# lzhangbj/ASVA

Measured on AMD Instinct MI355X. Metric: UNet denoising steps/sec, 12x256x256 bf16, CFG on, higher is better.
Workload: dtype bf16; 1 GPU; BASELINE configs[1]: AVSync15 shape, 1 clip(s) per GPU per forward, 12x256x256 (latent 12x32x32), SD1.5-shaped AudioUNet3D 1.17B params random-init, CFG batch 2 (audio guidance 4.0), DDIM-50 schedule, step = UNet forward + guidance + scheduler update; clips_per_gpu=1, unet_batch=2, frames=12, launch=hipGraph replay, parallelism=dp1 (independent clips)

## Files before the change

asva_amd/_lib.py:

```python
from __future__ import annotations

import ctypes as C
import os

import torch

from . import precision as P

_HERE = os.path.dirname(os.path.abspath(__file__))
LIB_PATH = os.environ.get("AVSD_LIB_PATH") or os.path.join(_HERE, "libavsd_hip.so")
LIB_PATHS = {"bf16": LIB_PATH, "fp16": os.environ.get("AVSD_LIB_PATH_F16") or os.path.join(_HERE, "libavsd_hip_f16.so")}

c_void_p, c_int, c_float, c_int64 = C.c_void_p, C.c_int, C.c_float, C.c_int64


class GemmDesc(C.Structure):

    _fields_ = [
        ("A", c_void_p), ("A2", c_void_p), ("W", c_void_p), ("out", c_void_p),
        ("bias", c_void_p), ("rowvec", c_void_p), ("res1", c_void_p), ("res2", c_void_p),
        ("M", C.c_int32), ("N", C.c_int32), ("K", C.c_int32),
        ("lda", C.c_int32), ("lda2", C.c_int32), ("k_split", C.c_int32), ("ldw", C.c_int32),
        ("ldc", C.c_int32), ("ldr1", C.c_int32), ("ldr2", C.c_int32),
        ("rows_per_vec", C.c_int32), ("ldv", C.c_int32),
# ... 40 lines not shown
    "avsd_gemm_bf16": (c_int, [C.POINTER(GemmDesc), c_void_p]),
    "avsd_sizeof_gemm_desc": (c_int, []),
    "avsd_cross_attention_block": (c_int, [C.POINTER(XAttnDesc), c_void_p]),
    "avsd_gemm_conv3r_supported": (c_int, [c_int, c_int, c_int, c_int]),
    "avsd_gemm_conv3r2d_supported": (c_int, [c_int, c_int, c_int, c_int]),
    "avsd_cross_attention_block_supported": (c_int, [c_int, c_int, c_int]),
    "avsd_sizeof_xattn_desc": (c_int, []),
    "avsd_qproj_attention": (c_int, [C.POINTER(XAttnDesc), c_void_p]),
    "avsd_qproj_attention_supported": (c_int, [c_int, c_int, c_int, c_int]),
    "avsd_ff_block": (c_int, [c_void_p, c_int, c_void_p, c_int, c_float, c_void_p, c_void_p, c_void_p, c_void_p, c_void_p, c_void_p, c_void_p,
                              c_void_p, c_int, c_void_p, c_int, c_int, c_int, c_void_p]),
    "avsd_ff_block_supported": (c_int, [c_int, c_int, c_int]),
    "avsd_temporal_block": (c_int, [c_void_p, c_int, c_void_p, c_int, c_float, c_void_p, c_void_p, c_void_p, c_void_p, c_void_p, c_void_p,
                                    c_void_p, c_int, c_void_p, c_int, c_int, c_int, c_int, c_int, c_float, c_void_p]),
    "avsd_temporal_block_supported": (c_int, [c_int, c_int, c_int, c_int]),
    "avsd_linear_small_m": (c_int, [c_void_p, c_void_p, c_void_p, c_void_p, c_int, c_int, c_int, c_int, c_int, c_int, c_void_p]),
    "avsd_groupnorm_stats": (c_int, [c_void_p, c_int, c_int, c_void_p, c_int, c_int, c_int, c_int, c_int, c_void_p, c_int, c_void_p]),
    "avsd_groupnorm_apply": (c_int, [c_void_p, c_int, c_int, c_void_p, c_int, c_int, c_int, c_int, c_int, c_void_p, c_void_p, c_float,
                                     c_void_p, c_int, c_int, c_void_p, c_int, c_void_p]),
    "avsd_ln_fold": (c_int, [c_void_p, c_int, c_int, c_void_p, c_void_p]),
    "avsd_groupnorm_fused_supported": (c_int, [c_int, c_int, c_int, c_int, c_int, c_int]),
    "avsd_groupnorm_fused": (c_int, [c_void_p, c_int, c_int, c_void_p, c_int, c_int, c_int, c_int, c_int, c_void_p, c_void_p, c_float,
                                     c_int, c_void_p, c_int, c_void_p]),
    "avsd_groupnorm_nchunks": (c_int, [c_int, c_int, c_int]),
    "avsd_groupnorm_scratch_floats": (c_int, [c_int, c_int, c_int, c_int]),
    "avsd_layernorm": (c_int, [c_void_p, c_int, c_void_p, c_int, c_int, c_int, c_void_p, c_void_p, c_float, c_void_p, c_int, c_int, c_void_p]),
    "avsd_softmax_rows": (c_int, [c_void_p, c_int, c_void_p, c_int, c_int, c_int, c_void_p]),
    "avsd_attention": (c_int, [c_void_p, c_int, c_void_p, c_int, c_void_p, c_int, c_void_p, c_int, c_int, c_int, c_int, c_int,
                               c_int, c_int, c_int, c_void_p, c_int, c_float, c_void_p]),
    "avsd_attention_fp8": (c_int, [c_void_p, c_int, c_void_p, c_int, c_void_p, c_int, c_void_p, c_int, c_int, c_int, c_int, c_int,
# ... 129 lines not shown
```

asva_amd/build.py:

```python
from __future__ import annotations

import os
import subprocess
import sys
from concurrent.futures import ThreadPoolExecutor

HERE = os.path.dirname(os.path.abspath(__file__))
CSRC = os.path.join(HERE, "csrc")
OBJ = os.path.join(CSRC, "_obj")
LIB = os.path.join(HERE, "libavsd_hip.so")
VARIANTS = {"bf16": ("", LIB, []), "fp16": ("_f16", os.path.join(HERE, "libavsd_hip_f16.so"), ["-DAVSD_F16=1"])}
SOURCES = ["lib.hip", "attention.hip", "attention_x2.hip", "gemm_f32.hip", "gemm4.hip", "nstream.hip", "conv3r.hip", "norm.hip", "groupnorm_fused.hip", "elementwise.hip", "audio.hip", "xattn.hip", "qattn.hip", "ffblock.hip", "tblock.hip", "attention_fp8.hip", "avsync.hip", "clip_text.hip", "imagebind_eval.hip", "jpeg.hip", "loss.hip", "plan.hip"]
GEMM_UNITS = 7
HEADERS = [os.path.join(CSRC, "avsd_common.h"), os.path.join(CSRC, "gemm_common.h"), os.path.join(CSRC, "gemm4_loops.inc"), os.path.join(CSRC, "band_units.h"),
           os.path.join(HERE, "..", "include", "avsd.h")]
FLAGS = ["--offload-arch=gfx950", "-O3", "-std=c++17", "-fPIC", "-Wall", "-Wno-unused-function"]


PLAN_HOST = os.path.join(HERE, "plan_host")


def _hipcc() -> str:
    for cand in (os.environ.get("HIPCC"), "/opt/rocm/bin/hipcc", "hipcc"):
        if cand and (os.path.isabs(cand) and os.path.exists(cand) or not os.path.isabs(cand)):
            return cand
    raise RuntimeError("hipcc not found")

# ... 57 lines not shown
```

asva_amd/csrc/plan.hip:

```cpp
#include "avsd_common.h"

#include <stdio.h>
#include <string.h>

#include <string>
#include <type_traits>
#include <utility>
#include <vector>

namespace {

struct RArg {
  int64_t i = 0;
  double f = 0.0;
  void* p = nullptr;
};

template <class T>
T conv(const RArg& a) {
  if constexpr (std::is_pointer_v<T>) return reinterpret_cast<T>(a.p);
  else if constexpr (std::is_floating_point_v<T>) return static_cast<T>(a.f);
  else return static_cast<T>(a.i);
}
template <class... A, size_t... I>
// ... 14 lines not shown
  const char* name;
  thunk_t thunk;
  size_t desc_bytes;
};
#define AVSD_PLAN_ENTRY(fn) {#fn, [](const RArg* a, int n) { return call(&fn, a, n, #fn); }, 0}
#define AVSD_PLAN_ENTRY_DESC(fn, T) {#fn, [](const RArg* a, int n) { return call(&fn, a, n, #fn); }, sizeof(T)}
const Entry kEntries[] = {
    AVSD_PLAN_ENTRY_DESC(avsd_gemm_bf16, avsd_gemm_desc), AVSD_PLAN_ENTRY_DESC(avsd_cross_attention_block, avsd_xattn_desc), AVSD_PLAN_ENTRY(avsd_linear_small_m),
    AVSD_PLAN_ENTRY(avsd_groupnorm_stats),  AVSD_PLAN_ENTRY(avsd_groupnorm_apply),       AVSD_PLAN_ENTRY(avsd_layernorm),
    AVSD_PLAN_ENTRY(avsd_softmax_rows),     AVSD_PLAN_ENTRY(avsd_attention),             AVSD_PLAN_ENTRY(avsd_attention_fp8),
    AVSD_PLAN_ENTRY(avsd_temporal_attention), AVSD_PLAN_ENTRY(avsd_ncfhw_to_rows),       AVSD_PLAN_ENTRY(avsd_rows_to_ncfhw),
    AVSD_PLAN_ENTRY(avsd_timestep_embedding), AVSD_PLAN_ENTRY(avsd_guided_step),         AVSD_PLAN_ENTRY(avsd_vae_postprocess),
    AVSD_PLAN_ENTRY(avsd_vae_postprocess_u8), AVSD_PLAN_ENTRY(avsd_kaldi_fbank),         AVSD_PLAN_ENTRY(avsd_patchify),
    AVSD_PLAN_ENTRY(avsd_vit_tokens),       AVSD_PLAN_ENTRY(avsd_copy),                  AVSD_PLAN_ENTRY(avsd_xattn_pack_kv),
    AVSD_PLAN_ENTRY_DESC(avsd_qproj_attention, avsd_xattn_desc), AVSD_PLAN_ENTRY(avsd_ff_block), AVSD_PLAN_ENTRY(avsd_temporal_block),
    AVSD_PLAN_ENTRY(avsd_linear_small_m_x2), AVSD_PLAN_ENTRY(avsd_groupnorm_stats_x2),   AVSD_PLAN_ENTRY(avsd_groupnorm_apply_x2),
    AVSD_PLAN_ENTRY(avsd_layernorm_x2),     AVSD_PLAN_ENTRY(avsd_attention_x2),          AVSD_PLAN_ENTRY(avsd_temporal_attention_x2),
    AVSD_PLAN_ENTRY(avsd_ncfhw_to_rows_x2), AVSD_PLAN_ENTRY(avsd_split_f32),             AVSD_PLAN_ENTRY(avsd_vae_postprocess_x2),
    AVSD_PLAN_ENTRY(avsd_vae_postprocess_u8_x2), AVSD_PLAN_ENTRY(avsd_softmax_rows_x2),
    AVSD_PLAN_ENTRY(avsd_groupnorm_fused),  AVSD_PLAN_ENTRY(avsd_groupnorm_fused_x2),
    AVSD_PLAN_ENTRY(avsd_ln_fold),          AVSD_PLAN_ENTRY(avsd_guided_multistep),      AVSD_PLAN_ENTRY(avsd_guided_unipc),
    AVSD_PLAN_ENTRY(avsd_window_turnover),
    AVSD_PLAN_ENTRY(avsd_convnd_f32),       AVSD_PLAN_ENTRY(avsd_maxpool_hw_f32),        AVSD_PLAN_ENTRY(avsd_mean_rows_f32),
    AVSD_PLAN_ENTRY(avsd_resize_aa_normalize_f32),
    AVSD_PLAN_ENTRY(avsd_convnd_ld_f32),    AVSD_PLAN_ENTRY(avsd_pool3_hw_f32),
    AVSD_PLAN_ENTRY(avsd_conv3d_same_f32),  AVSD_PLAN_ENTRY(avsd_maxpool3d_same_f32),
    AVSD_PLAN_ENTRY(avsd_embed_tokens_f32), AVSD_PLAN_ENTRY(avsd_layernorm_f32),         AVSD_PLAN_ENTRY(avsd_attention_causal_f32),
    AVSD_PLAN_ENTRY(avsd_quick_gelu_f32),
    AVSD_PLAN_ENTRY(avsd_attention_f32),    AVSD_PLAN_ENTRY(avsd_gelu_f32),              AVSD_PLAN_ENTRY(avsd_vit_tokens_f32),
    AVSD_PLAN_ENTRY(avsd_cosine_rows_f32),   AVSD_PLAN_ENTRY(avsd_normalize_rows_f32),
// ... 376 lines not shown
```

asva_amd/ops.py:

```python
from __future__ import annotations

import os
import ctypes as C
from typing import Optional, Tuple

import torch

from . import _lib
from . import precision as P
from ._lib import GemmDesc, XAttnDesc, check

PLAIN, TMIX, CONV3 = 0, 1, 2
GEGLU, OUT_F32, GELU, XCD_N, ROWSTATS, LNFUSE, RES1_F32, RES2_F32, X2, KROT, W_FRAG, OUT_REST = 1, 2, 4, 8, 16, 32, 64, 128, 256, 512, 1024, 2048
_XCD_MODE = "auto"
F32 = torch.float32


class KernelTimer:

    def __init__(self):
        self.records = []
        self.replays = []

    def start(self):
# ... 760 lines not shown
    M, K = x.shape
    N = w.shape[0]
    if not x.is_contiguous():
        raise ValueError("linear_small_m: x must be contiguous")
    if out is None:
        out = torch.empty((M, N), dtype=F32, device=x.device)
    if P.SPLIT:
        check(_lib.lib().avsd_linear_small_m_x2(_p(x), _p(w), _lo(w), _p(bias), _p(out), M, N, K, _ld(w), int(act_in), int(act_out),
                                                _stream()), "avsd_linear_small_m_x2")
        return out
    check(_lib.lib().avsd_linear_small_m(_p(x), _p(w), _p(bias), _p(out), M, N, K, _ld(w), int(act_in), int(act_out),
                                         _stream()), "avsd_linear_small_m")
    return out


_GN_FUSED = True

def groupnorm(x1: torch.Tensor, x2: Optional[torch.Tensor], nb: int, rows_per_batch: int, groups: int,
              gamma: torch.Tensor, beta: torch.Tensor, eps: float, act: bool,
              out: Optional[torch.Tensor] = None) -> torch.Tensor:
    _req(x1, P.ACT, "x1")
    c1 = x1.shape[1]
    c2 = 0
    if x2 is not None:
        _req(x2, P.ACT, "x2")
        c2 = x2.shape[1]
    _req(gamma, F32, "gamma")
    _req(beta, F32, "beta")
    L = _lib.lib()
    rows = nb * rows_per_batch
    if out is None:
# ... 321 lines not shown
    if out is None:
        out = torch.empty((M, Cc), dtype=P.ACT, device=h.device)
    _req(out, P.ACT, "out")
    if out.shape != (M, Cc):
        raise ValueError("temporal_block: out must be [M, C]")
    if scale is None:
        scale = float(Cc // heads) ** -0.5
    a_ = (_p(h), _ld(h), _p(stats), int(stats.shape[1]), float(eps), _p(wqkv_frag), _p(qkv_colsum), _p(qkv_bias), _p(posw), _p(wo_frag),
          _p(bo), _p(out), _ld(out), _p(rowstats), b, frames, hw, Cc, heads, float(scale))
    _timed("temporal_block", 8.0 * M * Cc * Cc + 4.0 * M * frames * Cc, _nbytes(h, out, rowstats) + 2.0 * (nq + Cc) * Cc,
           (h, stats, wqkv_frag, qkv_colsum, qkv_bias, posw, wo_frag, bo, rowstats, out),
           lambda: check(_lib.lib().avsd_temporal_block(*a_, _stream()), "avsd_temporal_block"))
    return out


def temporal_attention(qkv: torch.Tensor, *, b: int, frames: int, hw: int, heads: int,
                       scale: Optional[float] = None, out: Optional[torch.Tensor] = None) -> torch.Tensor:
    _req(qkv, P.ACT, "qkv")
    Cc = qkv.shape[1] // 3
    d = Cc // heads
    if out is None:
        out = alloc16((qkv.shape[0], Cc), qkv.device)
    if scale is None:
        scale = float(d) ** -0.5
    if P.SPLIT:
        a_ = (_p(qkv), _ld(qkv), _lo(qkv), _p(out), _ld(out), _lo(out), b, frames, hw, heads, d, float(scale))
        call = lambda: check(_lib.lib().avsd_temporal_attention_x2(*a_, _stream()), "avsd_temporal_attention_x2")
    else:
        a_ = (_p(qkv), _ld(qkv), _p(out), _ld(out), b, frames, hw, heads, d, float(scale))
        call = lambda: check(_lib.lib().avsd_temporal_attention(*a_, _stream()), "avsd_temporal_attention")
# ... 711 lines not shown
```

asva_amd/plan.py:

```python
from __future__ import annotations

import contextlib
import ctypes as C
import os
import struct
from typing import Dict, List, Optional, Tuple

import torch

from . import _lib
from . import precision as P

CONST, INPUT, OUTPUT = 1, 2, 3
MAGIC = b"AVSDPLN1"
_NOT_RECORDED = {"avsd_abi_version", "avsd_precision", "avsd_last_error", "avsd_device_info", "avsd_sizeof_gemm_desc",
                 "avsd_sizeof_xattn_desc", "avsd_cross_attention_block_supported", "avsd_qproj_attention_supported", "avsd_ff_block_supported", "avsd_temporal_block_supported", "avsd_groupnorm_nchunks",
                 "avsd_groupnorm_scratch_floats", "avsd_groupnorm_fused_supported", "avsd_gemm_conv3r_supported", "avsd_gemm_conv3r2d_supported"}


def _ptr_fields(struct_type) -> List[Tuple[str, int]]:
    return [(name, getattr(struct_type, name).offset) for name, tp in struct_type._fields_ if tp is C.c_void_p]


class _Proxy:

    def __init__(self, real, sink):
        self._real, self._sink = real, sink

    def __getattr__(self, name):
        fn = getattr(self._real, name)
        if (name in _NOT_RECORDED or name.startswith("avsd_plan_") or name.startswith("avsd_unet_") or name == "avsd_vae_decode"
# ... 237 lines not shown
```

asva_amd/unet.py:

```python
from __future__ import annotations

import inspect
import json
import math
import os
from typing import Any, Dict, Optional, Tuple, Union

import torch
from torch import nn

from . import precision as P

from . import ops
from .conditioning import mask_to_key_index
from .weights import Blob, _Pk, _Ref, from_act, group_qkv, pack_conv1x1, pack_device, pack_frag, pack_geglu, pack_linear, subpixel_ups, to_act, to_planes

CONFIG_NAME = "config.json"
SAFETENSORS_NAME = "diffusion_pytorch_model.safetensors"
BIN_NAME = "diffusion_pytorch_model.bin"

DOWN_TYPES = ("FFSpatioAudioTempCrossAttnDownBlock3D", "FFSpatioTempCrossAttnDownBlock3D", "FFSpatioTempResDownBlock3D")
UP_TYPES = ("FFSpatioAudioTempCrossAttnUpBlock3D", "FFSpatioTempCrossAttnUpBlock3D", "FFSpatioTempResUpBlock3D")
MID_TYPES = ("FFSpatioAudioTempCrossAttnUNetMidBlock3D", "FFSpatioTempCrossAttnUNetMidBlock3D")


_FUSE_LN = True
_FUSE_LN_TEMP = True
_F32_RES = os.environ.get("AVSD_F32_RESIDUAL", "0") != "0"
_ATTN_FP8 = os.environ.get("AVSD_ATTN_FP8", "0") != "0"
_FUSE_XATTN = True
_FUSE_QATTN = os.environ.get("AVSD_FUSE_QATTN", "1") != "0"
_FUSE_FF = os.environ.get("AVSD_FUSE_FF", "1") != "0"
_FUSE_TATTN = os.environ.get("AVSD_FUSE_TATTN", "1") != "0"
_LN_PREFOLD = True
_SHARE_PREFIX = True
_F32_CONV_Y = True


def _replicate(a: "_Act", r: int) -> "_Act":
    return _Act(ops.copy(a.lo, rep=r), None if a.hi is None else ops.copy(a.hi, rep=r),
                None if a.rest is None else ops.copy(a.rest, rep=r))


def _xa_fill(kv: torch.Tensor, n_kv: int, rows: int, C: int, idx: Optional[torch.Tensor], old=None):
    nb, lk = (n_kv, rows) if idx is None else (n_kv * idx.shape[0], idx.shape[1])
    lkp = (lk + 31) // 32 * 32
    if lkp > 96 or P.SPLIT:
        return None
# ... 308 lines not shown
                w1_ln=reg(w1_ln), b1_ln=reg(b1_ln), s1_ln=reg(from_act(w1_ln).sum(1)),
                norm_temp=self.aff(b.norm_temp), attn_temp=self.attn(b.attn_temp, True, b.norm_temp),
                pos1=self.lin(b.pos_embedding_temp.linear_1), pos2=self.lin(b.pos_embedding_temp.linear_2),
                norm3=self.aff(b.norm3), w1=reg(w1), b1=reg(b1), ff2=self.lin(b.ff.net[2]),
                dim=m.proj_in.weight.shape[0], audio=hasattr(b, "attn_audio"))
        if w1_ln.shape[1] in (320, 640) and not P.SPLIT:
            p.w1_ln_f = reg(pack_frag(w1_ln))
            if p.dim == 320:
                p.w2_f = reg(pack_frag(self.items[p.ff2.w.idx]))
                p.wp_f = reg(pack_frag(self.items[p.proj_out.w.idx]))
        if p.dim == 320 and not P.SPLIT:
            at = p.attn_temp
            at.wqkv_f = reg(pack_frag(group_qkv(self.items[at.wqkv_ln.idx])))
            at.sqkv_f, at.bqkv_f = reg(group_qkv(self.items[at.sqkv_ln.idx])), reg(group_qkv(self.items[at.bqkv_ln.idx]))
            at.wo_f = reg(pack_frag(self.items[at.wo.idx]))
        if p.audio:
            p.norm_audio = self.aff(b.norm_audio)
            p.attn_audio = self.attn(b.attn_audio, False, b.norm_audio)
        return p

    def block(self, m: _Block, where: Optional[str] = None):
        return _Pk(resnets=[self.res(r, where) for r in m.resnets],
                   attentions=[self.tr(a) for a in m.attentions] if hasattr(m, "attentions") else None,
                   down=self.ffconv(m.downsamplers[0].conv, "sampler", where) if hasattr(m, "downsamplers") else None,
                   up=self.ffconv(m.upsamplers[0].conv, "sampler", where, subpixel=P.SUBPIXEL_UPS) if hasattr(m, "upsamplers") else None)

    def finish(self, pk: _Pk, device, meta: bool = False) -> _Pk:
        if self.temb_w:
            pk.temb_w = self.reg(pack_linear(torch.cat(self.temb_w, 0)))
            pk.temb_b = self.reg(torch.cat(self.temb_b, 0))
# ... 556 lines not shown
        assert skip is None
        s = x
    tv = st.temb[:, p.temb_off:p.temb_off + p.cout]
    a = ops.groupnorm(x.lo, None if skip is None else skip.lo, st.B, rows_b, st.groups, p.norm1.g, p.norm1.b, st.eps, True)
    h = _ffconv(st, _Act(a), p.conv1, hw, temb=tv, master=False)
    a2 = ops.groupnorm(h.lo, None, st.B, rows_b, st.groups, p.norm2.g, p.norm2.b, st.eps, True)
    return _ffconv(st, _Act(a2), p.conv2, hw, res=s, rest=rest)


def _transformer(st, x: _Act, p, hw, heads, split: int = 1, rest=False) -> _Act:
    B, Fr = st.B, st.F
    L = hw[0] * hw[1]
    C = p.dim
    c = st.cond.blocks[st.tr_i]
    st.tr_i += 1
    n = ops.groupnorm(x.lo, None, B * Fr, L, st.groups, p.norm.g, p.norm.b, 1e-6, False)
    fused = C % 32 == 0 and st.fuse_ln
    eps = 1e-5
    M = B * Fr * L
    stats = [torch.empty((M, C // 32, 2), dtype=torch.float32, device=n.device) for _ in range(2)] if fused else None
    si = 0

    def stream(a, w, bias, res, want_stats=True, stats_pos=None, rest=False):
        nonlocal si
        m = _master(st, a, w.shape[0])
        if fused and want_stats:
            si ^= 1
            return _Act(ops.gemm(a, w, bias=bias, res1=None if res is None else res.res, rowstats=stats[si], master=m, stats_pos=stats_pos), m)
        o16 = o16r = None
        if rest and m is not None:
            o16, o16r = ops.alloc_planes((a.shape[0], w.shape[0]), a.device)
        return _Act(ops.gemm(a, w, bias=bias, res1=None if res is None else res.res, master=m, out=o16, out_rest=o16r), m, o16r)

    def cross(h, a, norm, xa, want_stats, unfused, stats_pos=None):
        nonlocal si
        if fused and st.fp8 is None and xa is not None and ops.cross_attention_block_supported(C, heads, xa.k.shape[1], M, L):
# ... 7 lines not shown
                                            heads=heads, L=L, q_per_kv=xa.q_per_kv, eps=eps, rowstats=s_out, master=m, stats_pos=stats_pos)
            return _Act(out, m)
        qa_ok = getattr(ops, "qproj_attention_supported", None)
        if (_FUSE_QATTN and fused and st.fp8 is None and xa is not None and qa_ok is not None
                and qa_ok(C, heads, xa.k.shape[1], M, L, xa.q_per_kv)):
            o = ops.qproj_attention(h.lo, stats[si], a.wq_ln, a.sq_ln, a.bq_ln, xa.k, xa.vt, xa.lk, heads=heads, L=L,
                                    q_per_kv=xa.q_per_kv, eps=eps)
            return stream(o, a.wo, a.bo, h, want_stats=want_stats, stats_pos=stats_pos)
        return stream(unfused(), a.wo, a.bo, h, want_stats=want_stats, stats_pos=stats_pos)

    def proj(h, norm, wl, bl, sl, w_plain):
        if fused:
            return ops.gemm(h.lo, wl, bias=bl, ln=(stats[si], sl, eps))
        return ops.gemm(ops.layernorm(h.lo, norm.g, norm.b), w_plain)

    h = stream(n, p.proj_in.w, p.proj_in.b, None)
    a1 = p.attn1
    if fused:
        kv = ops.gemm_batched(h.lo.view(B, Fr * L, C)[:, :L], a1.wkv_ln.unsqueeze(0).expand(B, 2 * C, C), bias=a1.bkv_ln,
                              ln=(stats[si], a1.skv_ln, eps)).view(B * L, 2 * C)
        q = ops.gemm(h.lo, a1.wq_ln, bias=a1.bq_ln, ln=(stats[si], a1.sq_ln, eps))
    else:
        n1 = ops.layernorm(h.lo, p.norm1.g, p.norm1.b)
        q = ops.gemm(n1, a1.wq)
        kv = ops.gemm_batched(n1.view(B, Fr * L, C)[:, :L], a1.wkv.unsqueeze(0).expand(B, 2 * C, C)).view(B * L, 2 * C)
    o = ops.attention(q, kv[:, :C], kv[:, C:], bq=B * Fr, lq=L, lk=L, kv_rows=L, heads=heads, q_per_kv=Fr, frames=Fr, fp8=st.fp8)
    h = stream(o, a1.wo, a1.bo, h)
    if split > 1:
        h, x = _replicate(h, split), _replicate(x, split)
        st.B = B = B * split
        M = B * Fr * L
        if fused:
            cur = stats[si]
            stats = [torch.empty((M, C // 32, 2), dtype=torch.float32, device=n.device) for _ in range(2)]
            ops.copy(cur, stats[si], rep=split)
    if p.audio:
        aa = p.attn_audio

        def audio_attention():
            q = proj(h, p.norm_audio, getattr(aa, "wq_ln", None), getattr(aa, "bq_ln", None), getattr(aa, "sq_ln", None), aa.wq)
            idx = st.cond.key_index
            return ops.attention(q, c.audio_kv[:, :C], c.audio_kv[:, C:], bq=B * Fr, lq=L,
                                 lk=idx.shape[1] if idx is not None else c.audio_len, kv_rows=c.audio_len, heads=heads,
                                 q_per_kv=Fr if c.audio_pf == 1 else 1, frames=st.cond.idx_frames if idx is not None else Fr,
                                 key_index=idx, fp8=st.fp8)

        h = cross(h, aa, p.norm_audio, getattr(c, "xa_audio", None), True, audio_attention)
    a2 = p.attn2

# ... 42 lines not shown
```

include/avsd.h:

```cpp
#ifndef AVSD_H
#define AVSD_H

#include <stddef.h>
#include <stdint.h>

#ifdef __cplusplus
extern "C" {
#endif

#define AVSD_OK 0
#define AVSD_EINVAL (-1)
#define AVSD_ELAUNCH (-2)
#define AVSD_ENODEV (-3)

#define AVSD_ABI_VERSION 10

int avsd_abi_version(void);
const char* avsd_precision(void);
const char* avsd_last_error(void);
int avsd_device_info(char* name_host, int len, int* num_cu_host);

enum { AVSD_GEMM_PLAIN = 0, AVSD_GEMM_TMIX = 1, AVSD_GEMM_CONV3 = 2 };
enum { AVSD_GEMM_GEGLU = 1, AVSD_GEMM_OUT_F32 = 2, AVSD_GEMM_GELU = 4, AVSD_GEMM_XCD_N = 8, AVSD_GEMM_ROWSTATS = 16,
       AVSD_GEMM_LNFUSE = 32, AVSD_GEMM_RES1_F32 = 64, AVSD_GEMM_RES2_F32 = 128, AVSD_GEMM_X2 = 256, AVSD_GEMM_KROT = 512, AVSD_GEMM_W_FRAG = 1024,
// ... 74 lines not shown
int avsd_sizeof_xattn_desc(void);

int avsd_qproj_attention_supported(int C, int heads, int lk_pad, int rows_per_kv_block);
int avsd_qproj_attention(const avsd_xattn_desc* desc_host, void* stream);

int avsd_ff_block_supported(int M, int C, int with_proj_out);
int avsd_ff_block(const void* h, int ldh, const float* ln_stats, int ln_nblk, float ln_eps, const void* w1_frag, const float* w1_colsum,
                  const float* b1, const void* w2_frag, const float* b2, const void* wp_frag, const float* bp, const void* x, int ldx,
                  void* out, int ldo, int M, int C, void* stream);

int avsd_temporal_block_supported(int M, int C, int heads, int frames);
int avsd_temporal_block(const void* h, int ldh, const float* ln_stats, int ln_nblk, float ln_eps, const void* wqkv_frag,
                        const float* qkv_colsum, const float* qkv_bias, const float* posw, const void* wo_frag, const float* bo,
                        void* out, int ldo, float* rowstats, int B, int frames, int hw, int C, int heads, float scale, void* stream);

int avsd_linear_small_m(const float* x, const void* W_bf16, const float* bias, float* out,
                        int M, int N, int K, int ldw, int act_in, int act_out, void* stream);

int avsd_groupnorm_stats(const void* x1, int ld1, int c1, const void* x2, int ld2, int c2,
                         int nb, int rows_per_batch, int groups, float* scratch, int nchunks, void* stream);
int avsd_groupnorm_apply(const void* x1, int ld1, int c1, const void* x2, int ld2, int c2,
                         int nb, int rows_per_batch, int groups, const float* gamma, const float* beta, float eps,
                         const float* scratch, int nchunks, int act, void* y, int ldy, void* stream);
int avsd_groupnorm_fused_supported(int nb, int rows_per_batch, int groups, int c1, int c2, int split);
int avsd_groupnorm_fused(const void* x1, int ld1, int c1, const void* x2, int ld2, int c2, int nb, int rows_per_batch,
                         int groups, const float* gamma, const float* beta, float eps, int act, void* y, int ldy, void* stream);
int avsd_groupnorm_nchunks(int nb, int rows_per_batch, int channels);
int avsd_groupnorm_scratch_floats(int nb, int nchunks, int groups, int channels);

int avsd_ln_fold(const float* stats, int M, int nblk, float* out, void* stream);
// ... 182 lines not shown
```

Baseline: 92.89 steps/s.

## Fuse groupnorm apply, proj_in and LN-folded Q projection into one kernel

```diff
diff --git a/asva_amd/_lib.py b/asva_amd/_lib.py
--- a/asva_amd/_lib.py
+++ b/asva_amd/_lib.py
@@ -78,6 +78,9 @@
     "avsd_temporal_block": (c_int, [c_void_p, c_int, c_void_p, c_int, c_float, c_void_p, c_void_p, c_void_p, c_void_p, c_void_p, c_void_p,
                                     c_void_p, c_int, c_void_p, c_int, c_int, c_int, c_int, c_int, c_float, c_void_p]),
     "avsd_temporal_block_supported": (c_int, [c_int, c_int, c_int, c_int]),
+    "avsd_block_front": (c_int, [c_void_p, c_int, c_void_p, c_int, c_void_p, c_void_p, c_float, c_int, c_int, c_void_p, c_void_p, c_void_p,
+                                 c_void_p, c_void_p, c_float, c_void_p, c_int, c_void_p, c_void_p, c_int, c_int, c_int, c_void_p]),
+    "avsd_block_front_supported": (c_int, [c_int, c_int, c_int, c_int, c_int]),
     "avsd_linear_small_m": (c_int, [c_void_p, c_void_p, c_void_p, c_void_p, c_int, c_int, c_int, c_int, c_int, c_int, c_void_p]),
     "avsd_groupnorm_stats": (c_int, [c_void_p, c_int, c_int, c_void_p, c_int, c_int, c_int, c_int, c_int, c_void_p, c_int, c_void_p]),
     "avsd_groupnorm_apply": (c_int, [c_void_p, c_int, c_int, c_void_p, c_int, c_int, c_int, c_int, c_int, c_void_p, c_void_p, c_float,
diff --git a/asva_amd/build.py b/asva_amd/build.py
--- a/asva_amd/build.py
+++ b/asva_amd/build.py
@@ -10,7 +10,7 @@
 OBJ = os.path.join(CSRC, "_obj")
 LIB = os.path.join(HERE, "libavsd_hip.so")
 VARIANTS = {"bf16": ("", LIB, []), "fp16": ("_f16", os.path.join(HERE, "libavsd_hip_f16.so"), ["-DAVSD_F16=1"])}
-SOURCES = ["lib.hip", "attention.hip", "attention_x2.hip", "gemm_f32.hip", "gemm4.hip", "nstream.hip", "conv3r.hip", "norm.hip", "groupnorm_fused.hip", "elementwise.hip", "audio.hip", "xattn.hip", "qattn.hip", "ffblock.hip", "tblock.hip", "attention_fp8.hip", "avsync.hip", "clip_text.hip", "imagebind_eval.hip", "jpeg.hip", "loss.hip", "plan.hip"]
+SOURCES = ["lib.hip", "attention.hip", "attention_x2.hip", "gemm_f32.hip", "gemm4.hip", "nstream.hip", "conv3r.hip", "norm.hip", "groupnorm_fused.hip", "elementwise.hip", "audio.hip", "xattn.hip", "qattn.hip", "ffblock.hip", "tblock.hip", "fblock.hip", "attention_fp8.hip", "avsync.hip", "clip_text.hip", "imagebind_eval.hip", "jpeg.hip", "loss.hip", "plan.hip"]
 GEMM_UNITS = 7
 HEADERS = [os.path.join(CSRC, "avsd_common.h"), os.path.join(CSRC, "gemm_common.h"), os.path.join(CSRC, "gemm4_loops.inc"), os.path.join(CSRC, "band_units.h"),
            os.path.join(HERE, "..", "include", "avsd.h")]
diff --git a/asva_amd/csrc/fblock.hip b/asva_amd/csrc/fblock.hip
--- /dev/null
+++ b/asva_amd/csrc/fblock.hip
@@ -0,0 +1,320 @@
+#include "gemm_common.h"
+
+namespace {
+
+typedef unsigned u32x4b __attribute__((ext_vector_type(4)));
+
+struct fb_args {
+  const h16_t* x; int ldx;
+  const float* partial; int nchunks;
+  const float* gamma; const float* beta; float gn_eps;
+  int rpb;
+  const u32x4b* wpi; const float* bpi;
+  const u32x4b* wq; const float* q_colsum; const float* q_bias; float ln_eps;
+  h16_t* h; int ldh;
+  float* rowstats;
+  h16_t* q; int ldq;
+  int M;
+};
+
+constexpr int FR_C = 320, FR_G = 32, FR_CG = FR_C / FR_G, FR_RF = 3, FR_BM = 32 * FR_RF;
+constexpr int FR_KS = FR_C / 16;
+constexpr int FR_NBLK = FR_C / 32;
+constexpr int FR_MIN_RPB = 8, FR_MAXB = (FR_BM - 2) / FR_MIN_RPB + 2;
+constexpr int FR_PITCH = FR_C * 2 + 16;
+constexpr int FR_BAND = FR_BM * FR_PITCH;
+constexpr int FR_TABLE = FR_MAXB * 2 * FR_C * 4;
+constexpr int FR_STATS = FR_BM * FR_NBLK * 8;
+constexpr int FR_MR = FR_MAXB * FR_G * 8;
+constexpr size_t FR_LDS = (size_t)2 * FR_BAND + FR_STATS + FR_MR;
+static_assert(FR_MAXB == 13 && FR_TABLE <= FR_BAND && FR_BAND % 16 == 0 && FR_LDS <= 160 * 1024, "LDS carve");
+
+__device__ __forceinline__ void unit_pack(const float (&v)[16], uint4& lo, uint4& hi) {
+  unsigned x[2][2], y[2][2];
+#pragma unroll
+  for (int d = 0; d < 2; ++d) {
+    const auto e = __builtin_amdgcn_permlane32_swap(pack2h(v[0 + 2 * d], v[1 + 2 * d]), pack2h(v[8 + 2 * d], v[9 + 2 * d]), false, false);
+    const auto o = __builtin_amdgcn_permlane32_swap(pack2h(v[4 + 2 * d], v[5 + 2 * d]), pack2h(v[12 + 2 * d], v[13 + 2 * d]), false, false);
+    x[0][d] = e[0]; x[1][d] = e[1];
+    y[0][d] = o[0]; y[1][d] = o[1];
+  }
+  lo = make_uint4(x[0][0], x[0][1], x[1][0], x[1][1]);
+  hi = make_uint4(y[0][0], y[0][1], y[1][0], y[1][1]);
+}
+
+__global__ __launch_bounds__(512, 1) void fblock_kernel(const fb_args p) {
+  extern __shared__ __attribute__((aligned(16))) unsigned char smb[];
+  constexpr int KS = FR_KS, PITCH = FR_PITCH, RF = FR_RF;
+  constexpr int D2 = 4;
+  const int tid = threadIdx.x, lane = tid & 63;
+  const int wave = __builtin_amdgcn_readfirstlane(tid >> 6);
+  const int m0 = blockIdx.x * FR_BM;
+  unsigned char* const band_n = smb;
+  unsigned char* const band_h = smb + FR_BAND;
+  float* const table = reinterpret_cast<float*>(band_h);
+  float2* const lstats = reinterpret_cast<float2*>(smb + 2 * FR_BAND);
+  float2* const mr = reinterpret_cast<float2*>(smb + 2 * FR_BAND + FR_STATS);
+  const int c0 = wave;
+  const bool extra = wave < 6;
+  const int c1 = extra ? 8 + wave / 3 : 8, b1 = extra ? wave % 3 : 0;
+  const int bat0 = m0 / p.rpb;
+  const int nbat = min(m0 + FR_BM - 1, p.M - 1) / p.rpb - bat0 + 1;
+
+  u32x4b qa[D2], qb[D2];
+  auto prefetch = [&](const u32x4b* w, int ln) {
+    const u32x4b* wa = w + ln + (int64_t)c0 * KS * 64;
+    const u32x4b* wb = w + ln + (int64_t)c1 * KS * 64;
+#pragma unroll
+    for (int d = 0; d < D2; ++d) {
+      qa[d] = __builtin_nontemporal_load(wa + d * 64);
+      if (extra) qb[d] = __builtin_nontemporal_load(wb + d * 64);
+    }
+  };
+  prefetch(p.wpi, lane);
+  constexpr int V = FR_C / 8;
+  constexpr int NV = (FR_BM * V + 511) / 512;
+  uint4 xv[NV];
+#pragma unroll
+  for (int i = 0; i < NV; ++i) {
+    const int v = min(tid + i * 512, FR_BM * V - 1), r = v / V, c = v - r * V;
+    xv[i] = *reinterpret_cast<const uint4*>(p.x + (int64_t)min(m0 + r, p.M - 1) * p.ldx + c * 8);
+  }
+  {
+    const int sub = tid & 31, half = tid >> 5;
+    const int npair = nbat * FR_G;
+    const float2* part = reinterpret_cast<const float2*>(p.partial);
+    for (int p0 = 0; p0 < npair; p0 += 64) {
+      float2 u[4][2];
+      const float2* base[4];
+#pragma unroll
+      for (int j = 0; j < 4; ++j) {
+        const int pi = min(p0 + 16 * j + half, npair - 1), t = pi / FR_G, g = pi - t * FR_G;
+        base[j] = part + (int64_t)(bat0 + t) * p.nchunks * FR_G + g;
+#pragma unroll
+        for (int e = 0; e < 2; ++e) {
+          const int k = sub + 32 * e;
+          u[j][e] = k < p.nchunks ? base[j][(int64_t)k * FR_G] : make_float2(0.f, 0.f);
+        }
+      }
+#pragma unroll
+      for (int j = 0; j < 4; ++j) {
+        const int pi = p0 + 16 * j + half;
+        double a = 0.0, q = 0.0;
+#pragma unroll
+        for (int e = 0; e < 2; ++e)
+          if (sub + 32 * e < p.nchunks) { a += (double)u[j][e].x; q += (double)u[j][e].y; }
+        for (int k = sub + 64; k < p.nchunks; k += 32) {
+          const float2 w = base[j][(int64_t)k * FR_G];
+          a += (double)w.x;
+          q += (double)w.y;
+        }
+        for (int off = 16; off > 0; off >>= 1) {
+          a += __shfl_xor(a, off, 64);
+          q += __shfl_xor(q, off, 64);
+        }
+        if (sub == 0 && pi < npair) {
+          const double n = (double)p.rpb * FR_CG;
+          const double mean = a / n;
+          double var = q / n - mean * mean;
+          if (var < 0.0) var = 0.0;
+          mr[pi] = make_float2((float)mean, (float)(1.0 / sqrt(var + (double)p.gn_eps)));
+        }
+      }
+    }
+  }
+  __syncthreads();
+  for (int i = tid; i < nbat * FR_C; i += 512) {
+    const int t = i / FR_C, c = i - t * FR_C;
+    const float2 s = mr[t * FR_G + c / FR_CG];
+    const float smean = s.x, srstd = s.y;
+    const float sc = srstd * p.gamma[c];
+    table[t * 2 * FR_C + c] = sc;
+    table[t * 2 * FR_C + FR_C + c] = p.beta[c] - smean * sc;
+  }
+  __syncthreads();
+#pragma unroll
+  for (int i = 0; i < NV; ++i) {
+    const int v = tid + i * 512, r = v / V, c = v - r * V;
+    if (v < FR_BM * V) {
+      const float* ss = table + (min(m0 + r, p.M - 1) / p.rpb - bat0) * 2 * FR_C + c * 8;
+      const float4 s0 = *reinterpret_cast<const float4*>(ss), s1 = *reinterpret_cast<const float4*>(ss + 4);
+      const float4 h0 = *reinterpret_cast<const float4*>(ss + FR_C), h1 = *reinterpret_cast<const float4*>(ss + FR_C + 4);
+      const float sc[8] = {s0.x, s0.y, s0.z, s0.w, s1.x, s1.y, s1.z, s1.w};
+      const float sh[8] = {h0.x, h0.y, h0.z, h0.w, h1.x, h1.y, h1.z, h1.w};
+      float f[8];
+      unpack8(xv[i], f);
+#pragma unroll
+      for (int e = 0; e < 8; ++e) f[e] = fmaf(f[e], sc[e], sh[e]);
+      *reinterpret_cast<uint4*>(band_n + r * PITCH + c * 16) = pack8(f);
+    }
+  }
+  __syncthreads();
+
+  f32x16 acc[4];
+  auto project = [&](const unsigned char* band, const u32x4b* w, int ln) {
+    const unsigned char* arow = band + (ln & 31) * PITCH + (ln >> 5) * 16;
+    const unsigned char* arow1 = arow + b1 * 32 * PITCH;
+    const u32x4b* wa = w + ln + (int64_t)c0 * KS * 64;
+    const u32x4b* wb = w + ln + (int64_t)c1 * KS * 64;
+#pragma unroll
+    for (int u = 0; u < 4; ++u)
+#pragma unroll
+      for (int r = 0; r < 16; ++r) acc[u][r] = 0.f;
+#pragma unroll
+    for (int ks = 0; ks < KS; ++ks) {
+      __builtin_amdgcn_sched_barrier(0);
+      h16x8 hf[RF];
+#pragma unroll
+      for (int b = 0; b < RF; ++b) hf[b] = *reinterpret_cast<const h16x8*>(arow + b * 32 * PITCH + ks * 32);
+      const h16x8 wf = __builtin_bit_cast(h16x8, qa[ks % D2]);
+#pragma unroll
+      for (int b = 0; b < RF; ++b) acc[b] = mfma32x32x16(wf, hf[b], acc[b], 0, 0, 0);
+      if (ks + D2 < KS) qa[ks % D2] = __builtin_nontemporal_load(wa + (ks + D2) * 64);
+      if (extra) {
+        const h16x8 hx = *reinterpret_cast<const h16x8*>(arow1 + ks * 32);
+        acc[3] = mfma32x32x16(__builtin_bit_cast(h16x8, qb[ks % D2]), hx, acc[3], 0, 0, 0);
+        if (ks + D2 < KS) qb[ks % D2] = __builtin_nontemporal_load(wb + (ks + D2) * 64);
+      }
+    }
+    __builtin_amdgcn_sched_barrier(0);
+  };
+
+  project(band_n, p.wpi, lane);
+  {
+    int lanev = lane, m0v = m0;
+    asm volatile("" : "+v"(lanev), "+s"(m0v));
+    prefetch(p.wq, lanev);
+    const int frow = lanev & 31, hsel = (lanev >> 5) * 4;
+#pragma unroll
+    for (int u = 0; u < 4; ++u) {
+      if (u == 3 && !extra) break;
+      const int c = u < 3 ? c0 : c1, b = u < 3 ? u : b1;
+      float v[16];
+#pragma unroll
+      for (int q = 0; q < 4; ++q) {
+        const float4 bb = *reinterpret_cast<const float4*>(p.bpi + 32 * c + 8 * q + hsel);
+        v[4 * q] = acc[u][4 * q] + bb.x; v[4 * q + 1] = acc[u][4 * q + 1] + bb.y; v[4 * q + 2] = acc[u][4 * q + 2] + bb.z; v[4 * q + 3] = acc[u][4 * q + 3] + bb.w;
+      }
+      uint4 lo, hi;
+      unit_pack(v, lo, hi);
+      const int row = 32 * b + frow, m = m0v + row;
+      unsigned char* rp = band_h + row * PITCH + (32 * c + 4 * hsel) * 2;
+      *reinterpret_cast<uint4*>(rp) = lo;
+      *reinterpret_cast<uint4*>(rp + 16) = hi;
+      if (m < p.M) {
+        h16_t* op = p.h + (int64_t)m * p.ldh + 32 * c + 4 * hsel;
+        *reinterpret_cast<uint4*>(op) = lo;
+        *reinterpret_cast<uint4*>(op + 8) = hi;
+      }
+      float sm, sq;
+      const unsigned w8[8] = {lo.x, lo.y, lo.z, lo.w, hi.x, hi.y, hi.z, hi.w};
+      rowstats16(w8, nullptr, sm, sq);
+      const auto t = __builtin_amdgcn_permlane32_swap(__float_as_uint(sm), __float_as_uint(sm), false, false);
+      const auto s = __builtin_amdgcn_permlane32_swap(__float_as_uint(sq), __float_as_uint(sq), false, false);
+      if (hsel == 0) {
+        const float2 pr = make_float2(__uint_as_float(t[0]) + __uint_as_float(t[1]), __uint_as_float(s[0]) + __uint_as_float(s[1]));
+        lstats[row * FR_NBLK + c] = pr;
+        if (m < p.M) reinterpret_cast<float2*>(p.rowstats)[(int64_t)m * FR_NBLK + c] = pr;
+      }
+    }
+  }
+  __syncthreads();
+  float pre_ln[2 * RF];
+  {
+    int lanev = lane;
+    asm volatile("" : "+v"(lanev));
+#pragma unroll
+    for (int b = 0; b < RF; ++b) {
+      const float4* st = reinterpret_cast<const float4*>(lstats + (32 * b + (lanev & 31)) * FR_NBLK);
+      float sm = 0.f, sq = 0.f;
+#pragma unroll
+      for (int j = 0; j < FR_NBLK / 2; ++j) {
+        const float4 t = st[j];
+        sm += t.x; sq += t.y; sm += t.z; sq += t.w;
+      }
+      const float inv_k = 1.0f / (float)FR_C;
+      const float mean = sm * inv_k;
+      const float var = fmaxf(sq * inv_k - mean * mean, 0.f);
+      pre_ln[2 * b] = rsqrtf(var + p.ln_eps);
+      pre_ln[2 * b + 1] = mean * pre_ln[2 * b];
+    }
+  }
+  project(band_h, p.wq, lane);
+  {
+    int lanev = lane, m0v = m0;
+    asm volatile("" : "+v"(lanev), "+s"(m0v));
+    const int frow = lanev & 31, hsel = (lanev >> 5) * 4;
+#pragma unroll
+    for (int u = 0; u < 4; ++u) {
+      if (u == 3 && !extra) break;
+      const int c = u < 3 ? c0 : c1, b = u < 3 ? u : b1;
+      const float rstd = u < 3 ? pre_ln[2 * u] : (b1 == 0 ? pre_ln[0] : b1 == 1 ? pre_ln[2] : pre_ln[4]);
+      const float mrs = u < 3 ? pre_ln[2 * u + 1] : (b1 == 0 ? pre_ln[1] : b1 == 1 ? pre_ln[3] : pre_ln[5]);
+      float v[16];
+#pragma unroll
+      for (int q = 0; q < 4; ++q) {
+        const float4 cs = *reinterpret_cast<const float4*>(p.q_colsum + 32 * c + 8 * q + hsel);
+        const float4 bb = *reinterpret_cast<const float4*>(p.q_bias + 32 * c + 8 * q + hsel);
+        const float c4[4] = {cs.x, cs.y, cs.z, cs.w}, b4[4] = {bb.x, bb.y, bb.z, bb.w};
+#pragma unroll
+        for (int i = 0; i < 4; ++i) v[4 * q + i] = fmaf(acc[u][4 * q + i] + 0.f, rstd, -mrs * c4[i]) + b4[i];
+      }
+      uint4 lo, hi;
+      unit_pack(v, lo, hi);
+      const int m = m0v + 32 * b + frow;
+      if (m < p.M) {
+        h16_t* op = p.q + (int64_t)m * p.ldq + 32 * c + 4 * hsel;
+        *reinterpret_cast<uint4*>(op) = lo;
+        *reinterpret_cast<uint4*>(op + 8) = hi;
+      }
+    }
+  }
+}
+
+constexpr int FR_MIN_M = 24576;
+
+}
+
+extern "C" int avsd_block_front_supported(int M, int C, int groups, int rows_per_batch, int with_kv) {
+  if (with_kv) return 0;
+  return C == FR_C && groups == FR_G && rows_per_batch >= FR_MIN_RPB && M >= FR_MIN_M && M % rows_per_batch == 0 ? 1 : 0;
+}
+
+extern "C" int avsd_block_front(const void* x, int ldx, const float* gn_partial, int nchunks, const float* gamma, const float* beta,
+                                float gn_eps, int rows_per_batch, int groups, const void* wpi_frag, const float* bpi, const void* wq_frag,
+                                const float* q_colsum, const float* q_bias, float ln_eps, void* h, int ldh, float* rowstats, void* q, int ldq,
+                                int M, int C, void* stream) {
+  AVSD_REQUIRE(C == FR_C && groups == FR_G, "block_front: unsupported shape: built for C = 320 in 32 groups only, got C = %d, %d groups", C, groups);
+  AVSD_REQUIRE(M > 0 && rows_per_batch >= FR_MIN_RPB && M % rows_per_batch == 0,
+               "block_front: unsupported shape: M = %d must be whole batches of rows_per_batch = %d >= %d rows", M, rows_per_batch, FR_MIN_RPB);
+  AVSD_REQUIRE(nchunks > 0 && nchunks <= rows_per_batch, "block_front: unsupported shape: nchunks = %d", nchunks);
+  AVSD_REQUIRE(x && gn_partial && gamma && beta && wpi_frag && bpi && wq_frag && q_colsum && q_bias && h && rowstats && q, "block_front: null operand");
+  AVSD_REQUIRE(ldx >= C && ldh >= C && ldq >= C && ldx % 8 == 0 && ldh % 8 == 0 && ldq % 8 == 0,
+               "block_front: unsupported strides: ldx %d, ldh %d and ldq %d must be multiples of 8, at least C", ldx, ldh, ldq);
+  AVSD_REQUIRE(((uintptr_t)x | (uintptr_t)h | (uintptr_t)q | (uintptr_t)wpi_frag | (uintptr_t)wq_frag | (uintptr_t)bpi | (uintptr_t)q_colsum |
+                (uintptr_t)q_bias | (uintptr_t)gamma | (uintptr_t)beta | (uintptr_t)rowstats) % 16 == 0 && (uintptr_t)gn_partial % 8 == 0,
+               "block_front: operands must be 16-byte aligned");
+  static bool attr_set = false;
+  if (!attr_set) {
+    hipError_t e = hipFuncSetAttribute(reinterpret_cast<const void*>(&fblock_kernel), hipFuncAttributeMaxDynamicSharedMemorySize, (int)FR_LDS);
+    if (e != hipSuccess) {
+      avsd_set_error("block_front: hipFuncSetAttribute(%zu B LDS): %s", FR_LDS, hipGetErrorString(e));
+      return AVSD_ELAUNCH;
+    }
+    attr_set = true;
+  }
+  fb_args a;
+  a.x = reinterpret_cast<const h16_t*>(x); a.ldx = ldx;
+  a.partial = gn_partial; a.nchunks = nchunks;
+  a.gamma = gamma; a.beta = beta; a.gn_eps = gn_eps;
+  a.rpb = rows_per_batch;
+  a.wpi = reinterpret_cast<const u32x4b*>(wpi_frag); a.bpi = bpi;
+  a.wq = reinterpret_cast<const u32x4b*>(wq_frag); a.q_colsum = q_colsum; a.q_bias = q_bias; a.ln_eps = ln_eps;
+  a.h = reinterpret_cast<h16_t*>(h); a.ldh = ldh;
+  a.rowstats = rowstats;
+  a.q = reinterpret_cast<h16_t*>(q); a.ldq = ldq;
+  a.M = M;
+  hipLaunchKernelGGL(fblock_kernel, dim3((unsigned)((M + FR_BM - 1) / FR_BM)), dim3(512), FR_LDS, reinterpret_cast<hipStream_t>(stream), a);
+  AVSD_CHECK_LAUNCH("block_front launch");
+  return AVSD_OK;
+}
diff --git a/asva_amd/csrc/plan.hip b/asva_amd/csrc/plan.hip
--- a/asva_amd/csrc/plan.hip
+++ b/asva_amd/csrc/plan.hip
@@ -52,6 +52,7 @@
     AVSD_PLAN_ENTRY(avsd_vae_postprocess_u8), AVSD_PLAN_ENTRY(avsd_kaldi_fbank),         AVSD_PLAN_ENTRY(avsd_patchify),
     AVSD_PLAN_ENTRY(avsd_vit_tokens),       AVSD_PLAN_ENTRY(avsd_copy),                  AVSD_PLAN_ENTRY(avsd_xattn_pack_kv),
     AVSD_PLAN_ENTRY_DESC(avsd_qproj_attention, avsd_xattn_desc), AVSD_PLAN_ENTRY(avsd_ff_block), AVSD_PLAN_ENTRY(avsd_temporal_block),
+    AVSD_PLAN_ENTRY(avsd_block_front),
     AVSD_PLAN_ENTRY(avsd_linear_small_m_x2), AVSD_PLAN_ENTRY(avsd_groupnorm_stats_x2),   AVSD_PLAN_ENTRY(avsd_groupnorm_apply_x2),
     AVSD_PLAN_ENTRY(avsd_layernorm_x2),     AVSD_PLAN_ENTRY(avsd_attention_x2),          AVSD_PLAN_ENTRY(avsd_temporal_attention_x2),
     AVSD_PLAN_ENTRY(avsd_ncfhw_to_rows_x2), AVSD_PLAN_ENTRY(avsd_split_f32),             AVSD_PLAN_ENTRY(avsd_vae_postprocess_x2),
diff --git a/asva_amd/ops.py b/asva_amd/ops.py
--- a/asva_amd/ops.py
+++ b/asva_amd/ops.py
@@ -798,7 +798,7 @@
     return out
 
 
-_GN_FUSED = True
+_GN_FUSED = os.environ.get("AVSD_GN_FUSED", "1") != "0"
 
 def groupnorm(x1: torch.Tensor, x2: Optional[torch.Tensor], nb: int, rows_per_batch: int, groups: int,
               gamma: torch.Tensor, beta: torch.Tensor, eps: float, act: bool,
@@ -1150,6 +1150,68 @@
     return out
 
 
+def groupnorm_stats(x: torch.Tensor, nb: int, rows_per_batch: int, groups: int):
+    if P.SPLIT:
+        raise ValueError("groupnorm_stats: not built for split precision (ops.groupnorm runs the pair)")
+    _req(x, P.ACT, "x")
+    if x.dim() != 2 or x.shape[0] != nb * rows_per_batch:
+        raise ValueError("groupnorm_stats: x must be [nb * rows_per_batch, C]")
+    L = _lib.lib()
+    Cc = x.shape[1]
+    nchunks = L.avsd_groupnorm_nchunks(nb, rows_per_batch, Cc)
+    partial = torch.empty((L.avsd_groupnorm_scratch_floats(nb, nchunks, groups, Cc),), dtype=F32, device=x.device)
+    s_ = (_p(x), _ld(x), Cc, None, 0, 0, nb, rows_per_batch, groups, _p(partial), nchunks)
+    _timed("groupnorm", 0.0, _nbytes(x), (x, partial), lambda: check(L.avsd_groupnorm_stats(*s_, _stream()), "avsd_groupnorm_stats"))
+    return partial, nchunks
+
+
+def block_front_supported(M: int, C: int, groups: int, rows_per_batch: int, with_kv: bool = False) -> bool:
+    return not P.SPLIT and bool(_lib.lib().avsd_block_front_supported(M, C, groups, rows_per_batch, int(with_kv)))
+
+
+def block_front(x: torch.Tensor, partial: torch.Tensor, nchunks: int, gamma: torch.Tensor, beta: torch.Tensor, wpi_frag: torch.Tensor,
+                bpi: torch.Tensor, wq_frag: torch.Tensor, q_colsum: torch.Tensor, q_bias: torch.Tensor, *, rows_per_batch: int,
+                groups: int = 32, gn_eps: float = 1e-6, eps: float = 1e-5, h: Optional[torch.Tensor] = None,
+                rowstats: Optional[torch.Tensor] = None, q: Optional[torch.Tensor] = None):
+    if P.SPLIT:
+        raise ValueError("block_front: not built for split precision (use the separate kernels)")
+    _req(x, P.ACT, "x")
+    _req(partial, F32, "partial")
+    _req(wpi_frag, P.ACT, "wpi_frag")
+    _req(wq_frag, P.ACT, "wq_frag")
+    for t, nm in ((gamma, "gamma"), (beta, "beta"), (bpi, "bpi"), (q_colsum, "q_colsum"), (q_bias, "q_bias")):
+        _req(t, F32, nm)
+    if x.dim() != 2:
+        raise ValueError("block_front: x must be [M, C]")
+    M, Cc = x.shape
+    if rows_per_batch <= 0 or M % rows_per_batch:
+        raise ValueError("block_front: M must be whole batches of rows_per_batch rows")
+    if (not wpi_frag.is_contiguous() or not wq_frag.is_contiguous() or wpi_frag.numel() != Cc * Cc or wq_frag.numel() != Cc * Cc
+            or any(t.numel() != Cc or not t.is_contiguous() for t in (gamma, beta, bpi, q_colsum, q_bias))):
+        raise ValueError("block_front: wpi_frag and wq_frag [C / 32, C / 16, 64, 8] with gamma, beta, bpi, q_colsum, q_bias [C]")
+    if not partial.is_contiguous() or nchunks <= 0 or partial.numel() != (M // rows_per_batch) * nchunks * groups * 2:
+        raise ValueError("block_front: partial must be the contiguous f32 [nb, nchunks, groups, 2] that groupnorm_stats wrote")
+    if rowstats is None:
+        rowstats = torch.empty((M, Cc // 32, 2), dtype=F32, device=x.device)
+    _req(rowstats, F32, "rowstats")
+    if not rowstats.is_contiguous() or tuple(rowstats.shape) != (M, Cc // 32, 2):
+        raise ValueError("block_front: rowstats must be contiguous f32 [M, C / 32, 2]")
+    if h is None:
+        h = torch.empty((M, Cc), dtype=P.ACT, device=x.device)
+    if q is None:
+        q = torch.empty((M, Cc), dtype=P.ACT, device=x.device)
+    for t, nm in ((h, "h"), (q, "q")):
+        _req(t, P.ACT, nm)
+        if t.shape != (M, Cc):
+            raise ValueError(f"block_front: {nm} must be [M, C]")
+    a_ = (_p(x), _ld(x), _p(partial), int(nchunks), _p(gamma), _p(beta), float(gn_eps), int(rows_per_batch), int(groups), _p(wpi_frag), _p(bpi),
+          _p(wq_frag), _p(q_colsum), _p(q_bias), float(eps), _p(h), _ld(h), _p(rowstats), _p(q), _ld(q), M, Cc)
+    _timed("block_front", 4.0 * M * Cc * Cc, _nbytes(x, h, q, rowstats) + 4.0 * Cc * Cc,
+           (x, partial, gamma, beta, wpi_frag, bpi, wq_frag, q_colsum, q_bias, h, rowstats, q),
+           lambda: check(_lib.lib().avsd_block_front(*a_, _stream()), "avsd_block_front"))
+    return h, rowstats, q
+
+
 def temporal_attention(qkv: torch.Tensor, *, b: int, frames: int, hw: int, heads: int,
                        scale: Optional[float] = None, out: Optional[torch.Tensor] = None) -> torch.Tensor:
     _req(qkv, P.ACT, "qkv")
diff --git a/asva_amd/plan.py b/asva_amd/plan.py
--- a/asva_amd/plan.py
+++ b/asva_amd/plan.py
@@ -14,7 +14,7 @@
 CONST, INPUT, OUTPUT = 1, 2, 3
 MAGIC = b"AVSDPLN1"
 _NOT_RECORDED = {"avsd_abi_version", "avsd_precision", "avsd_last_error", "avsd_device_info", "avsd_sizeof_gemm_desc",
-                 "avsd_sizeof_xattn_desc", "avsd_cross_attention_block_supported", "avsd_qproj_attention_supported", "avsd_ff_block_supported", "avsd_temporal_block_supported", "avsd_groupnorm_nchunks",
+                 "avsd_sizeof_xattn_desc", "avsd_cross_attention_block_supported", "avsd_qproj_attention_supported", "avsd_ff_block_supported", "avsd_temporal_block_supported", "avsd_block_front_supported", "avsd_groupnorm_nchunks",
                  "avsd_groupnorm_scratch_floats", "avsd_groupnorm_fused_supported", "avsd_gemm_conv3r_supported", "avsd_gemm_conv3r2d_supported"}
 
 
diff --git a/asva_amd/unet.py b/asva_amd/unet.py
--- a/asva_amd/unet.py
+++ b/asva_amd/unet.py
@@ -32,6 +32,7 @@
 _FUSE_QATTN = os.environ.get("AVSD_FUSE_QATTN", "1") != "0"
 _FUSE_FF = os.environ.get("AVSD_FUSE_FF", "1") != "0"
 _FUSE_TATTN = os.environ.get("AVSD_FUSE_TATTN", "1") != "0"
+_FUSE_FRONT = os.environ.get("AVSD_FUSE_FRONT", "1") != "0"
 _LN_PREFOLD = True
 _SHARE_PREFIX = True
 _F32_CONV_Y = True
@@ -370,6 +371,8 @@
             at.wqkv_f = reg(pack_frag(group_qkv(self.items[at.wqkv_ln.idx])))
             at.sqkv_f, at.bqkv_f = reg(group_qkv(self.items[at.sqkv_ln.idx])), reg(group_qkv(self.items[at.bqkv_ln.idx]))
             at.wo_f = reg(pack_frag(self.items[at.wo.idx]))
+            p.wpi_f = reg(pack_frag(self.items[p.proj_in.w.idx]))
+            p.attn1.wq_f = reg(pack_frag(self.items[p.attn1.wq_ln.idx]))
         if p.audio:
             p.norm_audio = self.aff(b.norm_audio)
             p.attn_audio = self.attn(b.attn_audio, False, b.norm_audio)
@@ -956,12 +959,14 @@
     C = p.dim
     c = st.cond.blocks[st.tr_i]
     st.tr_i += 1
-    n = ops.groupnorm(x.lo, None, B * Fr, L, st.groups, p.norm.g, p.norm.b, 1e-6, False)
     fused = C % 32 == 0 and st.fuse_ln
     eps = 1e-5
     M = B * Fr * L
-    stats = [torch.empty((M, C // 32, 2), dtype=torch.float32, device=n.device) for _ in range(2)] if fused else None
+    stats = [torch.empty((M, C // 32, 2), dtype=torch.float32, device=x.lo.device) for _ in range(2)] if fused else None
     si = 0
+    bf_ok = getattr(ops, "block_front_supported", None)
+    front = (_FUSE_FRONT and fused and hasattr(p, "wpi_f") and not P.SPLIT and not st.f32_stream and P.PLAN is None and st.fp8 is None
+             and bf_ok is not None and bf_ok(M, C, st.groups, L))
 
     def stream(a, w, bias, res, want_stats=True, stats_pos=None, rest=False):
         nonlocal si
@@ -999,12 +1004,22 @@
             return ops.gemm(h.lo, wl, bias=bl, ln=(stats[si], sl, eps))
         return ops.gemm(ops.layernorm(h.lo, norm.g, norm.b), w_plain)
 
-    h = stream(n, p.proj_in.w, p.proj_in.b, None)
     a1 = p.attn1
+    q = None
+    if front:
+        partial, nchunks = ops.groupnorm_stats(x.lo, B * Fr, L, st.groups)
+        si ^= 1
+        h16, _, q = ops.block_front(x.lo, partial, nchunks, p.norm.g, p.norm.b, p.wpi_f, p.proj_in.b, a1.wq_f, a1.sq_ln, a1.bq_ln,
+                                    rows_per_batch=L, groups=st.groups, gn_eps=1e-6, eps=eps, rowstats=stats[si])
+        h = _Act(h16)
+    else:
+        n = ops.groupnorm(x.lo, None, B * Fr, L, st.groups, p.norm.g, p.norm.b, 1e-6, False)
+        h = stream(n, p.proj_in.w, p.proj_in.b, None)
     if fused:
         kv = ops.gemm_batched(h.lo.view(B, Fr * L, C)[:, :L], a1.wkv_ln.unsqueeze(0).expand(B, 2 * C, C), bias=a1.bkv_ln,
                               ln=(stats[si], a1.skv_ln, eps)).view(B * L, 2 * C)
-        q = ops.gemm(h.lo, a1.wq_ln, bias=a1.bq_ln, ln=(stats[si], a1.sq_ln, eps))
+        if q is None:
+            q = ops.gemm(h.lo, a1.wq_ln, bias=a1.bq_ln, ln=(stats[si], a1.sq_ln, eps))
     else:
         n1 = ops.layernorm(h.lo, p.norm1.g, p.norm1.b)
         q = ops.gemm(n1, a1.wq)
@@ -1017,7 +1032,7 @@
         M = B * Fr * L
         if fused:
             cur = stats[si]
-            stats = [torch.empty((M, C // 32, 2), dtype=torch.float32, device=n.device) for _ in range(2)]
+            stats = [torch.empty((M, C // 32, 2), dtype=torch.float32, device=h.lo.device) for _ in range(2)]
             ops.copy(cur, stats[si], rep=split)
     if p.audio:
         aa = p.attn_audio
diff --git a/include/avsd.h b/include/avsd.h
--- a/include/avsd.h
+++ b/include/avsd.h
@@ -112,6 +112,11 @@
                         const float* qkv_colsum, const float* qkv_bias, const float* posw, const void* wo_frag, const float* bo,
                         void* out, int ldo, float* rowstats, int B, int frames, int hw, int C, int heads, float scale, void* stream);
 
+int avsd_block_front_supported(int M, int C, int groups, int rows_per_batch, int with_kv);
+int avsd_block_front(const void* x, int ldx, const float* gn_partial, int nchunks, const float* gamma, const float* beta, float gn_eps,
+                     int rows_per_batch, int groups, const void* wpi_frag, const float* bpi, const void* wq_frag, const float* q_colsum,
+                     const float* q_bias, float ln_eps, void* h, int ldh, float* rowstats, void* q, int ldq, int M, int C, void* stream);
+
 int avsd_linear_small_m(const float* x, const void* W_bf16, const float* bias, float* out,
                         int M, int N, int K, int ldw, int act_in, int act_out, void* stream);
 
```

Result: no change. 93.21 steps/s, median of 6 (+0.3%).
